# Kateridge/TransMF_AD

Measured on AMD Instinct MI355X. Metric: volume-pairs/sec fwd+bwd(+Adam), 96^3 MRI+PET batch=8 per GPU, higher is better.
Workload: dtype f32

## Files before the change

transmf_ad_amd/csrc/conv1_gram.hip:

```cpp
#include "tmf_common.h"

namespace {

constexpr int GT_D = 8, GT_H = 8, GT_W = 32;
constexpr int GP_D = GT_D + 2, GP_H = GT_H + 4, GP_W = GT_W + 4;
constexpr int GTHR = 512, GWG = 256, NACC = 64;

__host__ __device__ constexpr int kidx(int dd, int dh, int dw) {
    return dd == 0 ? (dh == 0 ? dw : 3 + (dh - 1) * 5 + (dw + 2)) : 13 + ((dd - 1) * 5 + (dh + 2)) * 5 + (dw + 2);
}
static_assert(kidx(2, 2, 2) == 62, "63 offsets");

typedef double f64x2 __attribute__((ext_vector_type(2)));
__device__ __forceinline__ float rbf16(float v) { return __builtin_bit_cast(float, tmf_pack_bf16(v, 0.f) << 16); }

__global__ __launch_bounds__(GTHR) void c1_gram_kernel(const float* __restrict__ x, double* __restrict__ part,
                                                        int D, int H, int W, int tilesD, int tilesH, int tilesW, int ntiles, int round16) {
    constexpr int NT = GP_D * GP_H * GP_W, NS = NT > 8 * GTHR ? NT : 8 * GTHR;
    __shared__ __attribute__((aligned(16))) double smem[NS];
    double* tile = smem;
    double* red = smem;
    const int tid = threadIdx.x;
    const int g = tid & 7, hh = (tid >> 3) & 7, dd0 = tid >> 6;
    double acc[63];
#pragma unroll
    for (int k = 0; k < 63; ++k) acc[k] = 0.0;
    double ssum = 0.0;
    constexpr int NE = (NT + GTHR - 1) / GTHR;
    int pe[NE];
#pragma unroll
    for (int j = 0; j < NE; ++j) {
        const int e = tid + j * GTHR;
        pe[j] = e < NT ? (e % GP_W) | (((e / GP_W) % GP_H) << 8) | ((e / (GP_W * GP_H)) << 16) : -1;
    }
    float pre[NE];
    auto fetch = [&](int t) {
        int r = t;
        const int bw = r % tilesW; r /= tilesW;
        const int bh = r % tilesH; r /= tilesH;
        const int bd = r % tilesD;
        const int b = r / tilesD;
        const int d0 = bd * GT_D, h0 = bh * GT_H - 2, w0 = bw * GT_W - 2;
        const float* xb = x + (size_t)b * D * H * W;
#pragma unroll
        for (int j = 0; j < NE; ++j) {
            const int gd = d0 + (pe[j] >> 16), gh = h0 + ((pe[j] >> 8) & 255), gw = w0 + (pe[j] & 255);
            float v = 0.f;
            if (pe[j] >= 0 && gd < D && gh >= 0 && gh < H && gw >= 0 && gw < W) v = xb[((size_t)gd * H + gh) * W + gw];
            pre[j] = round16 ? rbf16(v) : v;
        }
    };
    if ((int)blockIdx.x < ntiles) fetch(blockIdx.x);
    for (int t = blockIdx.x; t < ntiles; t += gridDim.x) {
        __syncthreads();
#pragma unroll
        for (int j = 0; j < NE; ++j)
            if (pe[j] >= 0) tile[tid + j * GTHR] = (double)pre[j];
        __syncthreads();
        if (t + (int)gridDim.x < ntiles) fetch(t + gridDim.x);
        const double* base = tile + (dd0 * GP_H + hh + 2) * GP_W + 4 * g;
        double a[4];
        {
            double rd[8];
#pragma unroll
            for (int j = 0; j < 4; ++j) { const f64x2 p = *reinterpret_cast<const f64x2*>(base + 2 * j); rd[2 * j] = p[0]; rd[2 * j + 1] = p[1]; }
            a[0] = rd[2]; a[1] = rd[3]; a[2] = rd[4]; a[3] = rd[5];
            ssum += (a[0] + a[1]) + (a[2] + a[3]);
#pragma unroll
            for (int dw = 0; dw <= 2; ++dw)
#pragma unroll
                for (int i = 0; i < 4; ++i) acc[kidx(0, 0, dw)] = fma(a[i], rd[i + 2 + dw], acc[kidx(0, 0, dw)]);
        }
#pragma unroll
        for (int dd = 0; dd <= 2; ++dd)
#pragma unroll
            for (int dh = -2; dh <= 2; ++dh) {
                if (dd == 0 && dh <= 0) continue;
                const double* row = base + (dd * GP_H + dh) * GP_W;
                double rd[8];
#pragma unroll
                for (int j = 0; j < 4; ++j) { const f64x2 p = *reinterpret_cast<const f64x2*>(row + 2 * j); rd[2 * j] = p[0]; rd[2 * j + 1] = p[1]; }
#pragma unroll
                for (int dw = -2; dw <= 2; ++dw)
#pragma unroll
                    for (int i = 0; i < 4; ++i) acc[kidx(dd, dh, dw)] = fma(a[i], rd[i + 2 + dw], acc[kidx(dd, dh, dw)]);
            }
    }
    const int lane = tid & 63, kq = tid >> 6;
#pragma unroll
    for (int c = 0; c < 8; ++c) {
        __syncthreads();
#pragma unroll
        for (int q = 0; q < 8; ++q) {
            const int k = c * 8 + q;
            red[q * GTHR + tid] = k < 63 ? acc[k < 63 ? k : 0] : ssum;
        }
        __syncthreads();
        double s = 0.0;
#pragma unroll
        for (int m = 0; m < 8; ++m) s += red[kq * GTHR + m * 64 + lane];
#pragma unroll
        for (int o = 32; o > 0; o >>= 1) s += __shfl_xor(s, o);
        if (lane == 0) part[(size_t)blockIdx.x * NACC + c * 8 + kq] = s;
    }
}

constexpr int GMAXC = 64;

constexpr int NGRAM = 760;
constexpr int HWG = 64, HTHR = 256, HNB = 288, HPART = 96;
constexpr int HNE = (HNB * 9 + HTHR - 1) / HTHR;

__host__ __device__ constexpr int class_tap(int cls, int j) {
    const int ax = cls >> 1, fixed = (cls & 1) ? 0 : 2, a = j / 3, b = j % 3;
    return ax == 0 ? fixed * 9 + a * 3 + b : (ax == 1 ? a * 9 + fixed * 3 + b : a * 9 + b * 3 + fixed);
}

__global__ __launch_bounds__(HTHR) void c1_shell_gram_kernel(const float* __restrict__ x, double* __restrict__ part, int B, int D, int H, int W,
                                                              int round16) {
    __shared__ double xs[HNB * 9];
    __shared__ int vbase[HNB], vcrd[HNB];
    __shared__ double red[3 * 81];
    const int tid = threadIdx.x, cls = blockIdx.y, ax = cls >> 1, side = cls & 1;
    const int n1 = ax == 0 ? H + 2 : D, n2 = ax == 2 ? H : W + 2;
    const int per = n1 * n2, total = B * per;
    const int p = tid % 81, slice = tid / 81, pi = p / 9, pj = p % 9;
    int cv_[HNE], cdd[HNE], cdh[HNE], cdw[HNE];
#pragma unroll
    for (int k = 0; k < HNE; ++k) {
        const int e = tid + k * HTHR, vi = e / 9, j = e - vi * 9, tap = class_tap(cls, j);
        cv_[k] = e < HNB * 9 ? vi : -1;
        cdd[k] = tap / 9 - 2; cdh[k] = (tap / 3) % 3 - 2; cdw[k] = tap % 3 - 2;
    }
    double acc = 0.0, eacc = 0.0;
    for (int base = blockIdx.x * HNB; base < total; base += gridDim.x * HNB) {
        __syncthreads();
        for (int vt = tid; vt < HNB; vt += HTHR) {
            const int s_ = base + vt;
            int c = -1, off = 0;
            if (s_ < total) {
                const int b = s_ / per, q = s_ - b * per, q1 = q / n2, q2 = q - q1 * n2;
                int vd, vh, vw;
                if (ax == 0) { vd = side ? D : -1; vh = q1 - 1; vw = q2 - 1; }
                else if (ax == 1) { vh = side ? H : -1; vd = q1; vw = q2 - 1; }
                else { vw = side ? W : -1; vd = q1; vh = q2; }
                c = (vd + 1) | (vh + 1) << 10 | (vw + 1) << 20;
                off = b * D * H * W;
            }
            vcrd[vt] = c; vbase[vt] = off;
        }
        __syncthreads();
#pragma unroll
        for (int k = 0; k < HNE; ++k) {
            if (cv_[k] < 0) continue;
            const int c = vcrd[cv_[k]];
            float v = 0.f;
            if (c >= 0) {
                const int ud = (c & 1023) + cdd[k], uh = ((c >> 10) & 1023) + cdh[k], uw = (c >> 20) + cdw[k];
                if (ud >= 0 && ud < D && uh >= 0 && uh < H && uw >= 0 && uw < W) v = x[(size_t)vbase[cv_[k]] + ((size_t)ud * H + uh) * W + uw];
            }
            xs[tid + k * HTHR] = (double)(round16 ? rbf16(v) : v);
        }
        __syncthreads();
        if (slice < 3) {
#pragma unroll 8
            for (int vi = slice * (HNB / 3); vi < (slice + 1) * (HNB / 3); ++vi) {
                const double xa = xs[vi * 9 + pi];
                acc = fma(xa, xs[vi * 9 + pj], acc);
                eacc += pj == 0 ? xa : 0.0;
            }
        }
    }
    __shared__ double rede[3 * 9];
    __syncthreads();
    if (slice < 3) {
        red[slice * 81 + p] = acc;
        if (pj == 0) rede[slice * 9 + pi] = eacc;
    }
    __syncthreads();
    double* row = part + ((size_t)cls * gridDim.x + blockIdx.x) * HPART;
    if (tid < 81) row[tid] = (red[tid] + red[81 + tid]) + red[162 + tid];
    else if (tid < 90) row[tid] = (rede[tid - 81] + rede[9 + tid - 81]) + rede[18 + tid - 81];
}

__global__ __launch_bounds__(1024) void c1_gram2_finish_kernel(const float* __restrict__ w, const double* __restrict__ rpart, int ngram,
                                                                const double* __restrict__ hpart, int nh, double* __restrict__ gram,
                                                                float* __restrict__ out, int C, int round16) {
    __shared__ double ra[16 * NACC];
    __shared__ double R[NACC];
    __shared__ double Hc[6 * HPART];
    __shared__ double G[27 * 27 + 27];
    __shared__ float wsh[27 * GMAXC];
    __shared__ double rows[27 * GMAXC];
    const int tid = threadIdx.x;
    {
        const int k = tid & 63, rg = tid >> 6;
        double s = 0.0;
#pragma unroll 8
        for (int i = rg; i < ngram; i += 16) s += rpart[(size_t)i * NACC + k];
        ra[rg * NACC + k] = s;
    }
    for (int e = tid; e < 27 * C; e += 1024) wsh[e] = round16 ? rbf16(w[e]) : w[e];
    for (int e = tid; e < 6 * HPART; e += 1024) {
        const int cls = e / HPART, k = e - cls * HPART;
        double s0 = 0.0, s1_ = 0.0, s2_ = 0.0, s3 = 0.0;
        if (k < 90) {
            int i = 0;
            for (; i + 3 < nh; i += 4) {
                s0 += hpart[((size_t)cls * nh + i) * HPART + k]; s1_ += hpart[((size_t)cls * nh + i + 1) * HPART + k];
                s2_ += hpart[((size_t)cls * nh + i + 2) * HPART + k]; s3 += hpart[((size_t)cls * nh + i + 3) * HPART + k];
            }
            for (; i < nh; ++i) s0 += hpart[((size_t)cls * nh + i) * HPART + k];
        }
        Hc[e] = (s0 + s1_) + (s2_ + s3);
    }
    __syncthreads();
    if (tid < NACC) {
        double s = 0.0;
#pragma unroll
        for (int i = 0; i < 16; ++i) s += ra[i * NACC + tid];
        R[tid] = s;
    }
    __syncthreads();
    for (int e = tid; e < 27 * 27 + 27; e += 1024) {
        double v;
        if (e < 729) {
            const int t = e / 27, u = e - t * 27;
            int dd = u / 9 - t / 9, dh = (u / 3) % 3 - (t / 3) % 3, dw = u % 3 - t % 3;
            if (dd < 0 || (dd == 0 && (dh < 0 || (dh == 0 && dw < 0)))) { dd = -dd; dh = -dh; dw = -dw; }
            v = R[kidx(dd, dh, dw)];
            for (int cls = 0; cls < 6; ++cls)
                for (int i = 0; i < 9; ++i) {
                    if (class_tap(cls, i) != t) continue;
                    for (int j = 0; j < 9; ++j)
                        if (class_tap(cls, j) == u) v -= Hc[cls * HPART + i * 9 + j];
// ... 49 lines not shown
    for (int e = tid; e < 27 * C; e += 1024) wsh[e] = round16 ? rbf16(w[e]) : w[e];
    __syncthreads();
    for (int j = tid; j < 2 * C; j += 1024) {
        double s = 0.0;
#pragma unroll
        for (int rg = 0; rg < 16; ++rg) s += pa[rg * 2 * C + j];
        c01[j] = s / count;
        if (coef) coef[j] = (float)c01[j];
        if (j < C) { if (dbeta) dbeta[j] = (float)s; }
        else if (dgamma) dgamma[j - C] = (float)s;
    }
    __syncthreads();
    for (int e = tid; e < 27 * C; e += 1024) {
        const int t = e / C, c = e - t * C;
        double v = 0.0;
        for (int u = 0; u < 27; ++u) v = fma((double)wsh[u * C + c], gram[t * 27 + u], v);
        const double st = gram[729 + t], mu = mean[c], is = invstd[c];
        const double r = (double)scale[c] * ((double)dred[e] - c01[c] * st - c01[C + c] * is * (v - mu * st));
        if (dw_ref) dw[(size_t)c * 27 + t] = (float)r;
        else dw[e] = (float)r;
    }
}

int c1_gram_mode() { return tmf_opt(TMF_OPT_C1_GRAM); }

}

extern "C" size_t tmf_c1_gram_bytes(int B, int D, int H, int W, int C) {
    if (B <= 0 || D <= 0 || H <= 0 || W <= 0 || C <= 0 || !c1_gram_mode() || C > GMAXC) return 0;
    if ((long)B * D * H * W >= (1L << 31) || D >= 1022 || H >= 1022 || W >= 1022) return 0;
    if ((long)B * tmf_cdiv(D, GT_D) * tmf_cdiv(H, GT_H) * tmf_cdiv(W, GT_W) >= (1L << 31)) return 0;
    return ((size_t)NGRAM + (size_t)GWG * NACC + (size_t)6 * HWG * HPART) * 8;
}
extern "C" size_t tmf_c1_gram_bytes_bf16(int B, int D, int H, int W, int C) {
    return c1_gram_mode() == 2 ? tmf_c1_gram_bytes(B, D, H, W, C) : 0;
}

static int c1_stats_g(int round16, const float* x, const float* w, float* stat_partial, void* gram, size_t gram_bytes,
                      int B, int D, int H, int W, int C, void* stream) {
    TMF_REQUIRE_PTR(x); TMF_REQUIRE_PTR(w); TMF_REQUIRE_PTR(stat_partial); TMF_REQUIRE_PTR(gram);
    const size_t need = tmf_c1_gram_bytes(B, D, H, W, C);
    TMF_REQUIRE(need > 0, TMF_E_SHAPE, "tmf_c1_stats_g: not available for this shape / option (tmf_c1_gram_bytes() = 0)");
    TMF_REQUIRE(gram_bytes >= need, TMF_E_WORKSPACE, "tmf_c1_stats_g: gram buffer %zu B < required %zu B", gram_bytes, need);
    TMF_REQUIRE((long)B * D * H * W < (1L << 31) && D < 1022 && H < 1022 && W < 1022, TMF_E_SHAPE,
                "tmf_c1_stats_g: the batch exceeds 2^31 voxels or an axis 1021");
    const int tilesD = tmf_cdiv(D, GT_D), tilesH = tmf_cdiv(H, GT_H), tilesW = tmf_cdiv(W, GT_W);
    const long ntiles = (long)B * tilesD * tilesH * tilesW;
    TMF_REQUIRE(ntiles < (1L << 31), TMF_E_SHAPE, "tmf_c1_stats_g: too many bricks");
    const int ngram = (int)(ntiles < GWG ? ntiles : GWG);
    double* g = (double*)gram;
    double* rpart = g + NGRAM;
    double* hpart = rpart + (size_t)GWG * NACC;
    hipStream_t s = (hipStream_t)stream;
    hipLaunchKernelGGL(c1_gram_kernel, dim3(ngram), dim3(GTHR), 0, s, x, rpart, D, H, W, tilesD, tilesH, tilesW, (int)ntiles, round16);
    hipLaunchKernelGGL(c1_shell_gram_kernel, dim3(HWG, 6), dim3(HTHR), 0, s, x, hpart, B, D, H, W, round16);
    hipLaunchKernelGGL(c1_gram2_finish_kernel, dim3(1), dim3(1024), 0, s, w, (const double*)rpart, ngram, (const double*)hpart, HWG, g,
                       stat_partial, C, round16);
    return tmf_launch_result("tmf_c1_stats_g");
}
extern "C" int tmf_c1_stats_g(const float* x, const float* w, float* stat_partial, void* gram, size_t gram_bytes,
                              int B, int D, int H, int W, int C, void* stream) {
    return c1_stats_g(0, x, w, stat_partial, gram, gram_bytes, B, D, H, W, C, stream);
}
extern "C" int tmf_c1_stats_g_bf16(const float* x, const float* w, float* stat_partial, void* gram, size_t gram_bytes,
                                   int B, int D, int H, int W, int C, void* stream) {
    return c1_stats_g(1, x, w, stat_partial, gram, gram_bytes, B, D, H, W, C, stream);
}

int tmf_c1_bwd_fused_finish(const float* part, int nblk, const float* dred, const float* w, const void* gram, const float* scale,
                            const float* mean, const float* invstd, double count, float* dgamma, float* dbeta, float* dw, int C,
                            int dw_ref, int round16, void* stream, float* coef) {
    hipLaunchKernelGGL(c1_bwd_fused_finish_kernel, dim3(1), dim3(1024), 0, (hipStream_t)stream, part, nblk, dred, w, (const double*)gram,
                       scale, mean, invstd, count, dgamma, dbeta, dw, C, dw_ref, round16, coef);
    return tmf_launch_result("tmf_c1_bwd_fused(finish)");
}
```

transmf_ad_amd/csrc/token_gemm.hip:

```cpp
#include <type_traits>
#include "tmf_device.h"

namespace {

constexpr int TM = 16, TTHR = 256;

struct TokArgs {
    const float* A; const float* W; float* Y;
    int R, K, N;
    const float* ln_g; const float* ln_b; float eps; float* ln_mean; float* ln_rstd; float* ln_out;
    const float* bias; const float* res; float* pre;
    const float* gelu_h;
    const float* lnb_x; const float* lnb_mean; const float* lnb_rstd; const float* lnb_g;
    const float* add1; const float* add2;
    float* lnb_partial; float* colsum_partial; int partial_stride;
    const float* mask; float* Y2;
};

__device__ __forceinline__ float hsum(f32x4 v) { return v[0] + v[1] + v[2] + v[3]; }
__device__ __forceinline__ float hsum(f32x2 v) { return v[0] + v[1]; }
__device__ __forceinline__ f32x4 minus(f32x4 v, float mu) { return f32x4{v[0] - mu, v[1] - mu, v[2] - mu, v[3] - mu}; }
__device__ __forceinline__ f32x2 minus(f32x2 v, float mu) { return f32x2{v[0] - mu, v[1] - mu}; }
__device__ __forceinline__ float sumsq(f32x4 d) { return d[0] * d[0] + d[1] * d[1] + d[2] * d[2] + d[3] * d[3]; }
__device__ __forceinline__ float sumsq(f32x2 d) { return d[0] * d[0] + d[1] * d[1]; }
// ... 323 lines not shown
        if (masked) TMF_REQUIRE_PTR_FN(fn, dx_masked);
        a.lnb_x = ln_x; a.lnb_mean = ln_mean; a.lnb_rstd = ln_rstd; a.lnb_g = ln_gamma;
        if (K == 64) return launch_ln_bwd<1>(a, s, fn);
        if (K == 128) return launch_ln_bwd<2>(a, s, fn);
        return launch_ln_bwd<4>(a, s, fn);
    }
    if (gelu) {
        TMF_REQUIRE(!masked || (add1 == nullptr && add2 == nullptr && dx_masked == nullptr), TMF_E_SHAPE,
                    "%s: the GELU-gradient epilogue takes no add1, add2 or dx_masked", fn);
        return launch_wide_opt_mask<true, 0, EPI_GELU_GRAD>(a, s, fn, "(gelu)");
    }
    a.res = add1;
    TMF_REQUIRE(add2 == nullptr, TMF_E_SHAPE, "%s: add2 needs the LayerNorm epilogue", fn);
    return launch_wide<true, 0, EPI_PLAIN>(a, s, fn, "");
}

extern "C" int tmf_tok_linear_fwd(const float* x, const float* w, const float* bias, const float* residual, float* y,
                                  int R, int K, int Nout, const float* ln_gamma, const float* ln_beta, float eps,
                                  float* ln_mean, float* ln_rstd, float* ln_out, float* gelu_pre, void* stream) {
    return tmf_tok_linear_fwd_impl(x, w, bias, residual, y, R, K, Nout, ln_gamma, ln_beta, eps, ln_mean, ln_rstd, ln_out, gelu_pre,
                                   nullptr, stream);
}

extern "C" int tmf_tok_linear_bwd_input(const float* dy, const float* w, float* dx, int R, int Nout, int K,
                                        const float* gelu_pre, const float* ln_x, const float* ln_mean,
                                        const float* ln_rstd, const float* ln_gamma, const float* add1,
                                        const float* add2, float* ln_partial, float* bias_partial,
                                        int partial_stride, void* stream) {
    return tmf_tok_linear_bwd_input_impl(dy, w, dx, R, Nout, K, gelu_pre, ln_x, ln_mean, ln_rstd, ln_gamma, add1, add2, ln_partial,
                                         bias_partial, partial_stride, nullptr, nullptr, stream);
}

extern "C" int tmf_tok_linear_fwd_masked(const float* x, const float* w, const float* bias, const float* residual, float* y,
                                         int R, int K, int Nout, const float* ln_gamma, const float* ln_beta, float eps,
                                         float* ln_mean, float* ln_rstd, float* ln_out, float* gelu_pre, const float* mask,
                                         void* stream) {
    TMF_REQUIRE_PTR(x); TMF_REQUIRE_PTR(w); TMF_REQUIRE_PTR(y); TMF_REQUIRE_PTR(mask);
    return tmf_tok_linear_fwd_impl(x, w, bias, residual, y, R, K, Nout, ln_gamma, ln_beta, eps, ln_mean, ln_rstd, ln_out, gelu_pre,
                                   mask, stream);
}

extern "C" int tmf_tok_linear_bwd_input_masked(const float* dy, const float* w, float* dx, int R, int Nout, int K,
                                               const float* gelu_pre, const float* ln_x, const float* ln_mean,
                                               const float* ln_rstd, const float* ln_gamma, const float* add1,
                                               const float* add2, float* ln_partial, float* bias_partial,
                                               int partial_stride, const float* mask, float* dx_masked, void* stream) {
    TMF_REQUIRE_PTR(dy); TMF_REQUIRE_PTR(w); TMF_REQUIRE_PTR(dx); TMF_REQUIRE_PTR(mask);
    return tmf_tok_linear_bwd_input_impl(dy, w, dx, R, Nout, K, gelu_pre, ln_x, ln_mean, ln_rstd, ln_gamma, add1, add2, ln_partial,
                                         bias_partial, partial_stride, mask, dx_masked, stream);
}

namespace {

constexpr int WG_MAXP = 32, WG_NSPLIT = 8;
struct WgMulti {
    const float* dy[WG_MAXP]; const float* x[WG_MAXP]; float* dw[WG_MAXP];
    int R[WG_MAXP], N[WG_MAXP], K[WG_MAXP], tile0[WG_MAXP + 1], elem0[WG_MAXP + 1];
    int nprob;
};

__global__ __launch_bounds__(256, 2) void tok_wgrad_multi_kernel(const WgMulti p, float* __restrict__ partial, long total_elems) {
    __shared__ float red[3][32 * 32];
    const int tid = threadIdx.x, lane = tid & 63;
    const int wave = __builtin_amdgcn_readfirstlane(tid >> 6);
    const int l31 = lane & 31, hsel = lane >> 5;
    int q = 0;
    while (q + 1 < p.nprob && (int)blockIdx.x >= p.tile0[q + 1]) ++q;
    const int t = blockIdx.x - p.tile0[q];
    const int tiles_k = p.K[q] >> 5;
    const int n0 = (t / tiles_k) * 32, k0 = (t % tiles_k) * 32;
    const int R = p.R[q], N = p.N[q], K = p.K[q];
    int rows = (R + WG_NSPLIT - 1) / WG_NSPLIT;
    rows = (rows + 7) & ~7;
    const int rb = blockIdx.y * rows + wave * (rows >> 2);
    const float* dy = p.dy[q] + n0 + l31;
    const float* xx = p.x[q] + k0 + l31;
    f32x16 acc;
#pragma unroll
    for (int r = 0; r < 16; ++r) acc[r] = 0.f;
    const int steps = rows >> 3;
    constexpr int UB = 16;
    for (int s0 = 0; s0 < steps; s0 += UB) {
        float a[UB], b[UB];
#pragma unroll
        for (int u = 0; u < UB; ++u) {
            const int row = rb + 2 * (s0 + u) + hsel;
            const bool ok = (s0 + u) < steps && row < R;
            const int rr = ok ? row : 0;
            a[u] = dy[(size_t)rr * N];
            b[u] = xx[(size_t)rr * K];
            a[u] = ok ? a[u] : 0.f;
        }
#pragma unroll
        for (int u = 0; u < UB; ++u) acc = __builtin_amdgcn_mfma_f32_32x32x2f32(a[u], b[u], acc, 0, 0, 0);
    }
    if (wave > 0) {
#pragma unroll
        for (int r = 0; r < 16; ++r) red[wave - 1][((r & 3) + 8 * (r >> 2) + 4 * hsel) * 32 + l31] = acc[r];
    }
    __syncthreads();
    if (wave == 0) {
        float* dst = partial + (size_t)blockIdx.y * total_elems + p.elem0[q];
#pragma unroll
        for (int r = 0; r < 16; ++r) {
            const int i = (r & 3) + 8 * (r >> 2) + 4 * hsel;
            const float v = acc[r] + red[0][i * 32 + l31] + red[1][i * 32 + l31] + red[2][i * 32 + l31];
            dst[(size_t)(n0 + i) * K + k0 + l31] = v;
        }
    }
}

__global__ __launch_bounds__(256) void tok_wgrad_multi_reduce_kernel(const WgMulti p, const float* __restrict__ partial,
                                                                     long total_elems) {
    const long e = (long)blockIdx.x * 256 + threadIdx.x;
    if (e >= total_elems) return;
    float s = 0.f;
#pragma unroll
    for (int k = 0; k < WG_NSPLIT; ++k) s += partial[(size_t)k * total_elems + e];
    int q = 0;
    while (q + 1 < p.nprob && e >= p.elem0[q + 1]) ++q;
    p.dw[q][e - p.elem0[q]] = s;
}

int fill_multi(WgMulti& m, int nprob, const float* const* dy, const float* const* x, float* const* dw,
               const int* R, const int* N, const int* K, const char* fn) {
    TMF_REQUIRE(nprob > 0 && nprob <= WG_MAXP, TMF_E_SHAPE, "%s: 1..%d problems, got %d", fn, WG_MAXP, nprob);
    m.nprob = nprob;
    m.tile0[0] = 0; m.elem0[0] = 0;
    for (int q = 0; q < nprob; ++q) {
        TMF_REQUIRE(R[q] > 0 && N[q] > 0 && K[q] > 0 && N[q] % 32 == 0 && K[q] % 32 == 0, TMF_E_SHAPE,
                    "%s: problem %d: R=%d N=%d K=%d (N and K must be multiples of 32)", fn, q, R[q], N[q], K[q]);
        m.R[q] = R[q]; m.N[q] = N[q]; m.K[q] = K[q];
        if (dy) { m.dy[q] = dy[q]; m.x[q] = x[q]; m.dw[q] = dw[q]; }
        m.tile0[q + 1] = m.tile0[q] + (N[q] / 32) * (K[q] / 32);
        m.elem0[q + 1] = m.elem0[q] + N[q] * K[q];
    }
    return TMF_OK;
}

}

extern "C" size_t tmf_tok_wgrad_multi_workspace_bytes(int nprob, const int* N, const int* K) {
    if (nprob <= 0 || nprob > WG_MAXP || N == nullptr || K == nullptr) return 0;
    size_t e = 0;
    for (int q = 0; q < nprob; ++q) e += (size_t)N[q] * K[q];
    return e * WG_NSPLIT * 4;
}

extern "C" int tmf_tok_wgrad_multi(int nprob, const float* const* dy, const float* const* x, float* const* dw,
                                   const int* R, const int* N, const int* K, void* workspace, size_t workspace_bytes,
                                   void* stream) {
    TMF_REQUIRE_PTR(dy); TMF_REQUIRE_PTR(x); TMF_REQUIRE_PTR(dw); TMF_REQUIRE_PTR(R); TMF_REQUIRE_PTR(N); TMF_REQUIRE_PTR(K);
    TMF_REQUIRE_PTR(workspace);
    WgMulti m = {};
    int rc = fill_multi(m, nprob, dy, x, dw, R, N, K, "tmf_tok_wgrad_multi");
    if (rc) return rc;
    for (int q = 0; q < nprob; ++q) { TMF_REQUIRE_PTR(dy[q]); TMF_REQUIRE_PTR(x[q]); TMF_REQUIRE_PTR(dw[q]); }
    const size_t need = tmf_tok_wgrad_multi_workspace_bytes(nprob, N, K);
    TMF_REQUIRE(workspace_bytes >= need, TMF_E_WORKSPACE, "tmf_tok_wgrad_multi: workspace %zu B < required %zu B",
                workspace_bytes, need);
    const long total = m.elem0[nprob];
    hipStream_t s = (hipStream_t)stream;
    hipLaunchKernelGGL(tok_wgrad_multi_kernel, dim3(m.tile0[nprob], WG_NSPLIT), dim3(256), 0, s, m, (float*)workspace, total);
    if ((rc = tmf_launch_result("tmf_tok_wgrad_multi"))) return rc;
    hipLaunchKernelGGL(tok_wgrad_multi_reduce_kernel, dim3((unsigned)tmf_cdiv(total, 256L)), dim3(256), 0, s, m,
                       (const float*)workspace, total);
    return tmf_launch_result("tmf_tok_wgrad_multi(reduce)");
}
```

transmf_ad_amd/csrc/token_ops.hip:

```cpp
#include "tmf_device.h"

static thread_local char g_err[512] = "";

void tmf_set_error(const char* fmt, ...) {
    va_list ap;
    va_start(ap, fmt);
    vsnprintf(g_err, sizeof g_err, fmt, ap);
    va_end(ap);
}

extern "C" int tmf_version(void) { return 1; }
extern "C" const char* tmf_last_error_string(void) { return g_err; }

namespace {

constexpr int LN_MAXV = 8;

template <int VEC>
__global__ __launch_bounds__(256) void layernorm_fwd_kernel(
    const float* __restrict__ x, const float* __restrict__ gamma, const float* __restrict__ beta,
    const float* __restrict__ residual, float* __restrict__ y, float* __restrict__ mean, float* __restrict__ rstd,
    int rows, int dim, float eps) {
    const int lane = threadIdx.x & 63;
    const int row = blockIdx.x * 4 + (threadIdx.x >> 6);
// ... 53 lines not shown
                    s1 += g;
                    s2 += g * xh;
                    ag[u * VEC + q] += gr[i + q] * xh;
                    ab[u * VEC + q] += gr[i + q];
                }
            }
        }
        s1 = wave_sum(s1) / dim;
        s2 = wave_sum(s2) / dim;
        float* dr = dx + (size_t)row * dim;
#pragma unroll
        for (int u = 0; u < LN_MAXV; ++u) {
            const int i = (u * 64 + lane) * VEC;
            if (i < dim) {
#pragma unroll
                for (int q = 0; q < VEC; ++q) {
                    const float xh = (xr[i + q] - mu) * rs;
                    const float v = rs * (gr[i + q] * gamma[i + q] - s1 - xh * s2);
                    dr[i + q] = v;
                    if (MASK) dxm[(size_t)row * dim + i + q] = v * mask[(size_t)row * dim + i + q];
                }
            }
        }
    }
#pragma unroll
    for (int u = 0; u < LN_MAXV; ++u) {
        const int i = (u * 64 + lane) * VEC;
        if (i < dim) {
#pragma unroll
            for (int q = 0; q < VEC; ++q) {
                red[(wave * 2 + 0) * dim + i + q] = ag[u * VEC + q];
                red[(wave * 2 + 1) * dim + i + q] = ab[u * VEC + q];
            }
        }
    }
    __syncthreads();
    for (int e = threadIdx.x; e < 2 * dim; e += 256) {
        const float a = red[e] + red[2 * dim + e] + red[4 * dim + e] + red[6 * dim + e];
        partial[(size_t)blockIdx.x * 2 * dim + e] = a;
    }
}

__global__ __launch_bounds__(256) void mask_mul_kernel(const float* __restrict__ x, const float* __restrict__ mask,
                                                       float* __restrict__ y, long n) {
    const long i = ((long)blockIdx.x * 256 + threadIdx.x) * 4;
    if (i + 4 <= n) {
        const f32x4 a = *reinterpret_cast<const f32x4*>(x + i), m = *reinterpret_cast<const f32x4*>(mask + i);
        *reinterpret_cast<f32x4*>(y + i) = f32x4{a[0] * m[0], a[1] * m[1], a[2] * m[2], a[3] * m[3]};
    } else {
        for (long j = i; j < n; ++j) y[j] = x[j] * mask[j];
    }
}

__global__ __launch_bounds__(256) void token_pool_fwd_kernel(const float* __restrict__ mri, const float* __restrict__ pet,
                                                             float* __restrict__ cls, int32_t* __restrict__ argmax,
                                                             int B, int N, int dim) {
    __shared__ float ssum[4][64], smax[4][64];
    __shared__ int sarg[4][64];
    const int cgroups = (dim + 63) / 64;
    const int cg = blockIdx.x % cgroups, mod = (blockIdx.x / cgroups) % 2, b = blockIdx.x / (2 * cgroups);
    const int cl = threadIdx.x & 63, tl = threadIdx.x >> 6;
    const int c = cg * 64 + cl;
    float s = 0.f, mx = -INFINITY;
    int am = 0;
    if (c < dim) {
        const float* src = (mod == 0 ? mri : pet) + (size_t)b * N * dim + c;
        for (int n = tl; n < N; n += 4) {
            const float v = src[(size_t)n * dim];
            s += v;
            if (v > mx || v != v) { mx = v; am = n; }
        }
    }
    ssum[tl][cl] = s; smax[tl][cl] = mx; sarg[tl][cl] = am;
    __syncthreads();
    if (tl == 0 && c < dim) {
#pragma unroll
        for (int k = 1; k < 4; ++k) {
            s += ssum[k][cl];
            const float v = smax[k][cl];
            const int a = sarg[k][cl];
            if (v != v) {
                if (mx == mx || a > am) { mx = v; am = a; }
            } else if (mx == mx && (v > mx || (v == mx && a < am))) { mx = v; am = a; }
        }
        cls[(size_t)b * 4 * dim + mod * dim + c] = s / N;
        cls[(size_t)b * 4 * dim + (2 + mod) * dim + c] = mx;
        argmax[((size_t)b * 2 + mod) * dim + c] = am;
    }
}

__global__ void token_pool_bwd_kernel(const float* __restrict__ dcls, const int32_t* __restrict__ argmax,
                                      float* __restrict__ dmri, float* __restrict__ dpet, int B, int N, int dim) {
    const long i = (long)blockIdx.x * blockDim.x + threadIdx.x;
    const long total = (long)B * 2 * N * dim;
    if (i >= total) return;
    const int c = i % dim;
    const int n = (i / dim) % N;
    const int mod = (i / ((long)dim * N)) % 2;
    const int b = i / ((long)dim * N * 2);
    const float gavg = dcls[(size_t)b * 4 * dim + mod * dim + c];
    const float gmax = dcls[(size_t)b * 4 * dim + (2 + mod) * dim + c];
    const int am = argmax[((size_t)b * 2 + mod) * dim + c];
    float* dst = (mod == 0 ? dmri : dpet);
    dst[((size_t)b * N + n) * dim + c] = gavg / N + (n == am ? gmax : 0.f);
}

__global__ __launch_bounds__(256) void pack_conv_weights_kernel(const float* __restrict__ w, float* __restrict__ fwd,
                                                                float* __restrict__ dgrad, int cout, int cin, int T) {
    const long n = (long)cout * cin * T;
    long e = (long)blockIdx.x * 256 + threadIdx.x;
    if (fwd != nullptr) {
        if (e < n) {
            const int co = e % cout, ci = (e / cout) % cin, t = e / ((long)cout * cin);
            fwd[e] = w[((long)co * cin + ci) * T + t];
            return;
        }
        e -= n;
    }
    if (dgrad != nullptr && e < n) {
        const int ci = e % cin, co = (e / cin) % cout, tr = e / ((long)cout * cin);
        dgrad[e] = w[((long)co * cin + ci) * T + (T - 1 - tr)];
    }
}

__global__ __launch_bounds__(256) void pack_conv_weights_bf16_kernel(const float* __restrict__ w, unsigned int* __restrict__ fwd,
                                                                     unsigned int* __restrict__ dgrad, int cout, int cin, int T) {
    const long n2 = (long)cout * cin * T / 2;
    long p = (long)blockIdx.x * 256 + threadIdx.x;
    if (p < n2) {
        const long e = 2 * p;
// ... 122 lines not shown

extern "C" int tmf_layernorm_bwd_blocks(int rows, int dim) {
    (void)dim;
    if (rows <= 0) return 0;
    return tmf_cdiv(rows, ln_rows_per_block(rows));
}

int tmf_layernorm_bwd_impl(const float* x, const float* gamma, const float* mean, const float* rstd, const float* dy, float* dx,
                           float* partial, int rows, int dim, const float* mask, float* dx_masked, void* stream) {
    const char* fn = mask != nullptr ? "tmf_layernorm_bwd_masked" : "tmf_layernorm_bwd";
    TMF_REQUIRE_PTR_FN(fn, x); TMF_REQUIRE_PTR_FN(fn, gamma); TMF_REQUIRE_PTR_FN(fn, mean); TMF_REQUIRE_PTR_FN(fn, rstd);
    TMF_REQUIRE_PTR_FN(fn, dy); TMF_REQUIRE_PTR_FN(fn, dx); TMF_REQUIRE_PTR_FN(fn, partial);
    if (mask != nullptr) TMF_REQUIRE_PTR_FN(fn, dx_masked);
    TMF_REQUIRE(rows > 0 && dim > 0, TMF_E_SHAPE, "%s: rows=%d dim=%d", fn, rows, dim);
    const int vec = dim % 4 == 0 ? 4 : 1;
    TMF_REQUIRE(dim <= 64 * vec * LN_MAXV, TMF_E_SHAPE, "%s: dim=%d exceeds %d", fn, dim, 64 * vec * LN_MAXV);
    const int rpb = ln_rows_per_block(rows);
    dim3 grid(tmf_cdiv(rows, rpb)), block(256);
    const size_t lds = (size_t)8 * dim * 4;
    if (mask == nullptr) dx_masked = nullptr;
    auto launch = [&](auto kernel) {
        hipLaunchKernelGGL(kernel, grid, block, lds, (hipStream_t)stream, x, gamma, mean, rstd, dy, dx, partial, rows, dim, rpb, mask, dx_masked);
    };
    if (mask != nullptr) vec == 4 ? launch(layernorm_bwd_kernel<4, true>) : launch(layernorm_bwd_kernel<1, true>);
    else                 vec == 4 ? launch(layernorm_bwd_kernel<4, false>) : launch(layernorm_bwd_kernel<1, false>);
    return tmf_launch_result(fn);
}

extern "C" int tmf_layernorm_bwd(const float* x, const float* gamma, const float* mean, const float* rstd,
                                 const float* dy, float* dx, float* partial, int rows, int dim, void* stream) {
    return tmf_layernorm_bwd_impl(x, gamma, mean, rstd, dy, dx, partial, rows, dim, nullptr, nullptr, stream);
}

extern "C" int tmf_layernorm_bwd_masked(const float* x, const float* gamma, const float* mean, const float* rstd,
                                        const float* dy, float* dx, float* partial, int rows, int dim,
                                        const float* mask, float* dx_masked, void* stream) {
    TMF_REQUIRE_PTR(x); TMF_REQUIRE_PTR(gamma); TMF_REQUIRE_PTR(mean); TMF_REQUIRE_PTR(rstd);
    TMF_REQUIRE_PTR(dy); TMF_REQUIRE_PTR(dx); TMF_REQUIRE_PTR(partial); TMF_REQUIRE_PTR(mask);
    return tmf_layernorm_bwd_impl(x, gamma, mean, rstd, dy, dx, partial, rows, dim, mask, dx_masked, stream);
}

extern "C" int tmf_mask_mul(const float* x, const float* mask, float* y, long n, void* stream) {
    TMF_REQUIRE_PTR(x); TMF_REQUIRE_PTR(mask); TMF_REQUIRE_PTR(y);
    TMF_REQUIRE_ALIGNED(x); TMF_REQUIRE_ALIGNED(mask); TMF_REQUIRE_ALIGNED(y);
    TMF_REQUIRE(n > 0 && n < (1L << 40), TMF_E_SHAPE, "tmf_mask_mul: n=%ld", n);
    hipLaunchKernelGGL(mask_mul_kernel, dim3((unsigned)tmf_cdiv(n, 1024L)), dim3(256), 0, (hipStream_t)stream, x, mask, y, n);
    return tmf_launch_result("tmf_mask_mul");
}

extern "C" int tmf_token_pool_fwd(const float* mri, const float* pet, float* cls, int32_t* argmax,
                                  int B, int N, int dim, void* stream) {
    TMF_REQUIRE_PTR(mri); TMF_REQUIRE_PTR(pet); TMF_REQUIRE_PTR(cls); TMF_REQUIRE_PTR(argmax);
    TMF_REQUIRE(B > 0 && N > 0 && dim > 0, TMF_E_SHAPE, "tmf_token_pool_fwd: B=%d N=%d dim=%d", B, N, dim);
    hipLaunchKernelGGL(token_pool_fwd_kernel, dim3(B * 2 * tmf_cdiv(dim, 64)), dim3(256), 0, (hipStream_t)stream,
                       mri, pet, cls, argmax, B, N, dim);
    return tmf_launch_result("tmf_token_pool_fwd");
}

extern "C" int tmf_token_pool_bwd(const float* dcls, const int32_t* argmax, float* dmri, float* dpet,
                                  int B, int N, int dim, void* stream) {
    TMF_REQUIRE_PTR(dcls); TMF_REQUIRE_PTR(argmax); TMF_REQUIRE_PTR(dmri); TMF_REQUIRE_PTR(dpet);
    TMF_REQUIRE(B > 0 && N > 0 && dim > 0, TMF_E_SHAPE, "tmf_token_pool_bwd: B=%d N=%d dim=%d", B, N, dim);
    const long total = (long)B * 2 * N * dim;
    hipLaunchKernelGGL(token_pool_bwd_kernel, dim3(tmf_cdiv(total, 256)), dim3(256), 0, (hipStream_t)stream,
                       dcls, argmax, dmri, dpet, B, N, dim);
    return tmf_launch_result("tmf_token_pool_bwd");
}
```

Baseline: 1029.

## Fuse conv1 gram kernels, retile token wgrad with LDS double-buffering, widen token pooling

The conv1 interior-gram and shell-gram kernels are merged into one launch. Its workgroups take either role, with each 512-thread group running two shell workgroups, so the two stages overlap and one launch is saved. The token weight-gradient GEMM moves to 64x64 tiles staged through double-buffered LDS with vectorized loads. Its split-K count is now adaptive, and the reduce pass is skipped when there is no split. Token pooling uses more threads per channel group with batched loads to raise memory-level parallelism. The changes raise LDS use and code complexity in exchange.

```diff
diff --git a/transmf_ad_amd/csrc/conv1_gram.hip b/transmf_ad_amd/csrc/conv1_gram.hip
--- a/transmf_ad_amd/csrc/conv1_gram.hip
+++ b/transmf_ad_amd/csrc/conv1_gram.hip
@@ -14,10 +14,15 @@
 typedef double f64x2 __attribute__((ext_vector_type(2)));
 __device__ __forceinline__ float rbf16(float v) { return __builtin_bit_cast(float, tmf_pack_bf16(v, 0.f) << 16); }
 
-__global__ __launch_bounds__(GTHR) void c1_gram_kernel(const float* __restrict__ x, double* __restrict__ part,
-                                                        int D, int H, int W, int tilesD, int tilesH, int tilesW, int ntiles, int round16) {
-    constexpr int NT = GP_D * GP_H * GP_W, NS = NT > 8 * GTHR ? NT : 8 * GTHR;
-    __shared__ __attribute__((aligned(16))) double smem[NS];
+constexpr int G_NT = GP_D * GP_H * GP_W, G_NS = G_NT > 8 * GTHR ? G_NT : 8 * GTHR;
+constexpr int HNB = 288;
+constexpr int H_NS = HNB * 9 + HNB + 3 * 81 + 3 * 9;
+constexpr int GS_NS = G_NS > 2 * H_NS ? G_NS : 2 * H_NS;
+
+__device__ __forceinline__ void c1_gram_role(double* __restrict__ smem, int blk, int nblk, const float* __restrict__ x,
+                                             double* __restrict__ part, int D, int H, int W, int tilesD, int tilesH, int tilesW,
+                                             int ntiles, int round16) {
+    constexpr int NT = G_NT;
     double* tile = smem;
     double* red = smem;
     const int tid = threadIdx.x;
@@ -50,14 +55,14 @@
             pre[j] = round16 ? rbf16(v) : v;
         }
     };
-    if ((int)blockIdx.x < ntiles) fetch(blockIdx.x);
-    for (int t = blockIdx.x; t < ntiles; t += gridDim.x) {
+    if (blk < ntiles) fetch(blk);
+    for (int t = blk; t < ntiles; t += nblk) {
         __syncthreads();
 #pragma unroll
         for (int j = 0; j < NE; ++j)
             if (pe[j] >= 0) tile[tid + j * GTHR] = (double)pre[j];
         __syncthreads();
-        if (t + (int)gridDim.x < ntiles) fetch(t + gridDim.x);
+        if (t + nblk < ntiles) fetch(t + nblk);
         const double* base = tile + (dd0 * GP_H + hh + 2) * GP_W + 4 * g;
         double a[4];
         {
@@ -101,27 +106,32 @@
         for (int m = 0; m < 8; ++m) s += red[kq * GTHR + m * 64 + lane];
 #pragma unroll
         for (int o = 32; o > 0; o >>= 1) s += __shfl_xor(s, o);
-        if (lane == 0) part[(size_t)blockIdx.x * NACC + c * 8 + kq] = s;
+        if (lane == 0) part[(size_t)blk * NACC + c * 8 + kq] = s;
     }
 }
 
 constexpr int GMAXC = 64;
 
 constexpr int NGRAM = 760;
-constexpr int HWG = 64, HTHR = 256, HNB = 288, HPART = 96;
+constexpr int HWG = 64, HTHR = 256, HPART = 96;
 constexpr int HNE = (HNB * 9 + HTHR - 1) / HTHR;
+static_assert(GTHR == 2 * HTHR && HWG % 2 == 0, "a 512-thread workgroup of the launch is a pair of shell workgroups");
 
 __host__ __device__ constexpr int class_tap(int cls, int j) {
     const int ax = cls >> 1, fixed = (cls & 1) ? 0 : 2, a = j / 3, b = j % 3;
     return ax == 0 ? fixed * 9 + a * 3 + b : (ax == 1 ? a * 9 + fixed * 3 + b : a * 9 + b * 3 + fixed);
 }
 
-__global__ __launch_bounds__(HTHR) void c1_shell_gram_kernel(const float* __restrict__ x, double* __restrict__ part, int B, int D, int H, int W,
-                                                              int round16) {
-    __shared__ double xs[HNB * 9];
-    __shared__ int vbase[HNB], vcrd[HNB];
-    __shared__ double red[3 * 81];
-    const int tid = threadIdx.x, cls = blockIdx.y, ax = cls >> 1, side = cls & 1;
+__device__ __forceinline__ void c1_shell_role(double* __restrict__ smem, int cls, int pair, const float* __restrict__ x,
+                                              double* __restrict__ part, int B, int D, int H, int W, int round16) {
+    const int half = threadIdx.x / HTHR, blk = 2 * pair + half;
+    smem += half * H_NS;
+    double* xs = smem;
+    int* vbase = reinterpret_cast<int*>(smem + HNB * 9);
+    int* vcrd = vbase + HNB;
+    double* red = smem + HNB * 9 + HNB;
+    double* rede = red + 3 * 81;
+    const int tid = threadIdx.x % HTHR, ax = cls >> 1, side = cls & 1;
     const int n1 = ax == 0 ? H + 2 : D, n2 = ax == 2 ? H : W + 2;
     const int per = n1 * n2, total = B * per;
     const int p = tid % 81, slice = tid / 81, pi = p / 9, pj = p % 9;
@@ -133,9 +143,11 @@
         cdd[k] = tap / 9 - 2; cdh[k] = (tap / 3) % 3 - 2; cdw[k] = tap % 3 - 2;
     }
     double acc = 0.0, eacc = 0.0;
-    for (int base = blockIdx.x * HNB; base < total; base += gridDim.x * HNB) {
-        __syncthreads();
-        for (int vt = tid; vt < HNB; vt += HTHR) {
+    for (int base0 = 2 * pair * HNB; base0 < total; base0 += HWG * HNB) {
+        const int base = base0 + half * HNB;
+        const bool live = base < total;
+        __syncthreads();
+        for (int vt = tid; live && vt < HNB; vt += HTHR) {
             const int s_ = base + vt;
             int c = -1, off = 0;
             if (s_ < total) {
@@ -150,19 +162,24 @@
             vcrd[vt] = c; vbase[vt] = off;
         }
         __syncthreads();
-#pragma unroll
-        for (int k = 0; k < HNE; ++k) {
-            if (cv_[k] < 0) continue;
-            const int c = vcrd[cv_[k]];
-            float v = 0.f;
-            if (c >= 0) {
+        if (live) {
+            float gv[HNE];
+            bool gok[HNE];
+#pragma unroll
+            for (int k = 0; k < HNE; ++k) {
+                const int vi = cv_[k] < 0 ? 0 : cv_[k], c = vcrd[vi];
                 const int ud = (c & 1023) + cdd[k], uh = ((c >> 10) & 1023) + cdh[k], uw = (c >> 20) + cdw[k];
-                if (ud >= 0 && ud < D && uh >= 0 && uh < H && uw >= 0 && uw < W) v = x[(size_t)vbase[cv_[k]] + ((size_t)ud * H + uh) * W + uw];
-            }
-            xs[tid + k * HTHR] = (double)(round16 ? rbf16(v) : v);
-        }
-        __syncthreads();
-        if (slice < 3) {
+                gok[k] = cv_[k] >= 0 && c >= 0 && ud >= 0 && ud < D && uh >= 0 && uh < H && uw >= 0 && uw < W;
+                gv[k] = x[gok[k] ? (size_t)vbase[vi] + ((size_t)ud * H + uh) * W + uw : (size_t)0];
+            }
+#pragma unroll
+            for (int k = 0; k < HNE; ++k) {
+                const float v = gok[k] ? gv[k] : 0.f;
+                if (cv_[k] >= 0) xs[tid + k * HTHR] = (double)(round16 ? rbf16(v) : v);
+            }
+        }
+        __syncthreads();
+        if (live && slice < 3) {
 #pragma unroll 8
             for (int vi = slice * (HNB / 3); vi < (slice + 1) * (HNB / 3); ++vi) {
                 const double xa = xs[vi * 9 + pi];
@@ -171,16 +188,24 @@
             }
         }
     }
-    __shared__ double rede[3 * 9];
     __syncthreads();
     if (slice < 3) {
         red[slice * 81 + p] = acc;
         if (pj == 0) rede[slice * 9 + pi] = eacc;
     }
     __syncthreads();
-    double* row = part + ((size_t)cls * gridDim.x + blockIdx.x) * HPART;
+    double* row = part + ((size_t)cls * HWG + blk) * HPART;
     if (tid < 81) row[tid] = (red[tid] + red[81 + tid]) + red[162 + tid];
     else if (tid < 90) row[tid] = (rede[tid - 81] + rede[9 + tid - 81]) + rede[18 + tid - 81];
+}
+
+__global__ __launch_bounds__(GTHR) void c1_gram_kernel_and_c1_shell_gram_kernel(const float* __restrict__ x, double* __restrict__ rpart,
+                                                              double* __restrict__ hpart, int B, int D, int H, int W, int tilesD,
+                                                              int tilesH, int tilesW, int ntiles, int ngram, int round16) {
+    __shared__ __attribute__((aligned(16))) double smem[GS_NS];
+    const int bid = blockIdx.x;
+    if (bid < 3 * HWG) c1_shell_role(smem, bid / (HWG / 2), bid % (HWG / 2), x, hpart, B, D, H, W, round16);
+    else c1_gram_role(smem, bid - 3 * HWG, ngram, x, rpart, D, H, W, tilesD, tilesH, tilesW, ntiles, round16);
 }
 
 __global__ __launch_bounds__(1024) void c1_gram2_finish_kernel(const float* __restrict__ w, const double* __restrict__ rpart, int ngram,
@@ -336,8 +361,8 @@
     double* rpart = g + NGRAM;
     double* hpart = rpart + (size_t)GWG * NACC;
     hipStream_t s = (hipStream_t)stream;
-    hipLaunchKernelGGL(c1_gram_kernel, dim3(ngram), dim3(GTHR), 0, s, x, rpart, D, H, W, tilesD, tilesH, tilesW, (int)ntiles, round16);
-    hipLaunchKernelGGL(c1_shell_gram_kernel, dim3(HWG, 6), dim3(HTHR), 0, s, x, hpart, B, D, H, W, round16);
+    hipLaunchKernelGGL(c1_gram_kernel_and_c1_shell_gram_kernel, dim3(3 * HWG + ngram), dim3(GTHR), 0, s, x, rpart, hpart, B, D, H, W, tilesD, tilesH, tilesW,
+                       (int)ntiles, ngram, round16);
     hipLaunchKernelGGL(c1_gram2_finish_kernel, dim3(1), dim3(1024), 0, s, w, (const double*)rpart, ngram, (const double*)hpart, HWG, g,
                        stat_partial, C, round16);
     return tmf_launch_result("tmf_c1_stats_g");
diff --git a/transmf_ad_amd/csrc/token_gemm.hip b/transmf_ad_amd/csrc/token_gemm.hip
--- a/transmf_ad_amd/csrc/token_gemm.hip
+++ b/transmf_ad_amd/csrc/token_gemm.hip
@@ -399,74 +399,133 @@
 
 namespace {
 
-constexpr int WG_MAXP = 32, WG_NSPLIT = 8;
+constexpr int WG_MAXP = 32, WG_MAXSPLIT = 8, WG_T = 64, WG_ROWS = 32;
+constexpr int WG_FILL = 4 * 256;
 struct WgMulti {
     const float* dy[WG_MAXP]; const float* x[WG_MAXP]; float* dw[WG_MAXP];
     int R[WG_MAXP], N[WG_MAXP], K[WG_MAXP], tile0[WG_MAXP + 1], elem0[WG_MAXP + 1];
     int nprob;
 };
 
-__global__ __launch_bounds__(256, 2) void tok_wgrad_multi_kernel(const WgMulti p, float* __restrict__ partial, long total_elems) {
-    __shared__ float red[3][32 * 32];
+int wg_splits(int tiles, int max_rows) {
+    int s = tmf_cdiv(WG_FILL, tiles);
+    if (s > WG_MAXSPLIT) s = WG_MAXSPLIT;
+    const int by_rows = tmf_cdiv(max_rows, WG_ROWS);
+    if (s > by_rows) s = by_rows;
+    return s < 1 ? 1 : s;
+}
+
+template <bool VEC>
+__global__ __launch_bounds__(256, 2) void tok_wgrad_multi_kernel(const WgMulti p, float* __restrict__ partial, long total_elems,
+                                                                 int nsplit) {
+    __shared__ __attribute__((aligned(16))) float sa[2][WG_ROWS][WG_T], sb[2][WG_ROWS][WG_T];
     const int tid = threadIdx.x, lane = tid & 63;
     const int wave = __builtin_amdgcn_readfirstlane(tid >> 6);
     const int l31 = lane & 31, hsel = lane >> 5;
+    const int item = blockIdx.x;
     int q = 0;
-    while (q + 1 < p.nprob && (int)blockIdx.x >= p.tile0[q + 1]) ++q;
-    const int t = blockIdx.x - p.tile0[q];
-    const int tiles_k = p.K[q] >> 5;
-    const int n0 = (t / tiles_k) * 32, k0 = (t % tiles_k) * 32;
+    while (q + 1 < p.nprob && item >= p.tile0[q + 1] * nsplit) ++q;
     const int R = p.R[q], N = p.N[q], K = p.K[q];
-    int rows = (R + WG_NSPLIT - 1) / WG_NSPLIT;
+    const int tiles_k = (K + WG_T - 1) / WG_T, tiles_q = p.tile0[q + 1] - p.tile0[q];
+    const int split = (item - p.tile0[q] * nsplit) / tiles_q, t = (item - p.tile0[q] * nsplit) % tiles_q;
+    const int n0 = (t / tiles_k) * WG_T, k0 = (t % tiles_k) * WG_T;
+    int rows = (R + nsplit - 1) / nsplit;
     rows = (rows + 7) & ~7;
-    const int rb = blockIdx.y * rows + wave * (rows >> 2);
-    const float* dy = p.dy[q] + n0 + l31;
-    const float* xx = p.x[q] + k0 + l31;
+    const int rb = split * rows;
+    const int re = rb + rows < R ? rb + rows : R;
+    const int wn = wave >> 1, wk = wave & 1;
+    const bool active = n0 + wn * 32 < N && k0 + wk * 32 < K;
+    const int lr = tid >> 4, lc = (tid & 15) * 4;
+    const float* dy = p.dy[q] + (n0 + lc < N ? n0 + lc : 0);
+    const float* xx = p.x[q] + (k0 + lc < K ? k0 + lc : 0);
+    auto fetch = [&](int r0, f32x4 (&va)[2], f32x4 (&vb)[2]) {
+#pragma unroll
+        for (int i = 0; i < 2; ++i) {
+            const int row = r0 + lr + 16 * i;
+            const size_t rr = row < R ? row : R - 1;
+            const float* pa = dy + rr * N;
+            const float* pb = xx + rr * K;
+            if constexpr (VEC) {
+                va[i] = *reinterpret_cast<const f32x4*>(pa);
+                vb[i] = *reinterpret_cast<const f32x4*>(pb);
+            } else {
+                va[i] = f32x4{pa[0], pa[1], pa[2], pa[3]};
+                vb[i] = f32x4{pb[0], pb[1], pb[2], pb[3]};
+            }
+        }
+    };
+    auto stash = [&](int buf, const f32x4 (&va)[2], const f32x4 (&vb)[2]) {
+#pragma unroll
+        for (int i = 0; i < 2; ++i) {
+            *reinterpret_cast<f32x4*>(&sa[buf][lr + 16 * i][lc]) = va[i];
+            *reinterpret_cast<f32x4*>(&sb[buf][lr + 16 * i][lc]) = vb[i];
+        }
+    };
     f32x16 acc;
 #pragma unroll
     for (int r = 0; r < 16; ++r) acc[r] = 0.f;
-    const int steps = rows >> 3;
-    constexpr int UB = 16;
-    for (int s0 = 0; s0 < steps; s0 += UB) {
-        float a[UB], b[UB];
-#pragma unroll
-        for (int u = 0; u < UB; ++u) {
-            const int row = rb + 2 * (s0 + u) + hsel;
-            const bool ok = (s0 + u) < steps && row < R;
-            const int rr = ok ? row : 0;
-            a[u] = dy[(size_t)rr * N];
-            b[u] = xx[(size_t)rr * K];
-            a[u] = ok ? a[u] : 0.f;
-        }
-#pragma unroll
-        for (int u = 0; u < UB; ++u) acc = __builtin_amdgcn_mfma_f32_32x32x2f32(a[u], b[u], acc, 0, 0, 0);
-    }
-    if (wave > 0) {
-#pragma unroll
-        for (int r = 0; r < 16; ++r) red[wave - 1][((r & 3) + 8 * (r >> 2) + 4 * hsel) * 32 + l31] = acc[r];
-    }
-    __syncthreads();
-    if (wave == 0) {
-        float* dst = partial + (size_t)blockIdx.y * total_elems + p.elem0[q];
-#pragma unroll
-        for (int r = 0; r < 16; ++r) {
-            const int i = (r & 3) + 8 * (r >> 2) + 4 * hsel;
-            const float v = acc[r] + red[0][i * 32 + l31] + red[1][i * 32 + l31] + red[2][i * 32 + l31];
-            dst[(size_t)(n0 + i) * K + k0 + l31] = v;
-        }
-    }
-}
-
+    auto multiply = [&](int buf, int r0) {
+        const int left = re - r0;
+        if (!active || left <= 0) return;
+        const int steps = left >= WG_ROWS ? WG_ROWS / 2 : (left + 1) >> 1;
+        const float* a = &sa[buf][hsel][wn * 32 + l31];
+        const float* b = &sb[buf][hsel][wk * 32 + l31];
+        if (steps == WG_ROWS / 2) {
+#pragma unroll
+            for (int s = 0; s < WG_ROWS / 2; ++s)
+                acc = __builtin_amdgcn_mfma_f32_32x32x2f32(a[2 * s * WG_T], b[2 * s * WG_T], acc, 0, 0, 0);
+        } else {
+            for (int s = 0; s < steps; ++s) {
+                const bool ok = 2 * s + hsel < left;
+                acc = __builtin_amdgcn_mfma_f32_32x32x2f32(ok ? a[2 * s * WG_T] : 0.f, ok ? b[2 * s * WG_T] : 0.f, acc, 0, 0, 0);
+            }
+        }
+    };
+    f32x4 va0[2], vb0[2], va1[2], vb1[2];
+    fetch(rb, va0, vb0);
+    __builtin_amdgcn_sched_barrier(0);
+    fetch(rb + WG_ROWS, va1, vb1);
+    __builtin_amdgcn_sched_barrier(0);
+    for (int r0 = rb; r0 < re; r0 += 2 * WG_ROWS) {
+        stash(0, va0, vb0);
+        __syncthreads();
+        fetch(r0 + 2 * WG_ROWS, va0, vb0);
+        multiply(0, r0);
+        stash(1, va1, vb1);
+        __syncthreads();
+        fetch(r0 + 3 * WG_ROWS, va1, vb1);
+        multiply(1, r0 + WG_ROWS);
+    }
+    if (active) {
+        float* dst = nsplit == 1 ? p.dw[q] : partial + (size_t)split * total_elems + p.elem0[q];
+        dst += (size_t)(n0 + wn * 32) * K + k0 + wk * 32 + l31;
+#pragma unroll
+        for (int r = 0; r < 16; ++r) dst[(size_t)((r & 3) + 8 * (r >> 2) + 4 * hsel) * K] = acc[r];
+    }
+}
+
+template <bool VEC>
 __global__ __launch_bounds__(256) void tok_wgrad_multi_reduce_kernel(const WgMulti p, const float* __restrict__ partial,
-                                                                     long total_elems) {
-    const long e = (long)blockIdx.x * 256 + threadIdx.x;
+                                                                     long total_elems, int nsplit) {
+    const long e = ((long)blockIdx.x * 256 + threadIdx.x) * 4;
     if (e >= total_elems) return;
-    float s = 0.f;
-#pragma unroll
-    for (int k = 0; k < WG_NSPLIT; ++k) s += partial[(size_t)k * total_elems + e];
+    f32x4 v[WG_MAXSPLIT];
+#pragma unroll
+    for (int k = 0; k < WG_MAXSPLIT; ++k) {
+        const float* src = partial + (size_t)(k < nsplit ? k : 0) * total_elems + e;
+        if constexpr (VEC) v[k] = *reinterpret_cast<const f32x4*>(src);
+        else v[k] = f32x4{src[0], src[1], src[2], src[3]};
+    }
+    f32x4 s = v[0];
+#pragma unroll
+    for (int k = 1; k < WG_MAXSPLIT; ++k)
+        if (k < nsplit) s += v[k];
+    const long e0 = (long)blockIdx.x * 1024;
     int q = 0;
-    while (q + 1 < p.nprob && e >= p.elem0[q + 1]) ++q;
-    p.dw[q][e - p.elem0[q]] = s;
+    while (q + 1 < p.nprob && e0 >= p.elem0[q + 1]) ++q;
+    float* dst = p.dw[q] + (e - p.elem0[q]);
+    if constexpr (VEC) *reinterpret_cast<f32x4*>(dst) = s;
+    else { dst[0] = s[0]; dst[1] = s[1]; dst[2] = s[2]; dst[3] = s[3]; }
 }
 
 int fill_multi(WgMulti& m, int nprob, const float* const* dy, const float* const* x, float* const* dw,
@@ -479,7 +538,7 @@
                     "%s: problem %d: R=%d N=%d K=%d (N and K must be multiples of 32)", fn, q, R[q], N[q], K[q]);
         m.R[q] = R[q]; m.N[q] = N[q]; m.K[q] = K[q];
         if (dy) { m.dy[q] = dy[q]; m.x[q] = x[q]; m.dw[q] = dw[q]; }
-        m.tile0[q + 1] = m.tile0[q] + (N[q] / 32) * (K[q] / 32);
+        m.tile0[q + 1] = m.tile0[q] + tmf_cdiv(N[q], WG_T) * tmf_cdiv(K[q], WG_T);
         m.elem0[q + 1] = m.elem0[q] + N[q] * K[q];
     }
     return TMF_OK;
@@ -490,8 +549,14 @@
 extern "C" size_t tmf_tok_wgrad_multi_workspace_bytes(int nprob, const int* N, const int* K) {
     if (nprob <= 0 || nprob > WG_MAXP || N == nullptr || K == nullptr) return 0;
     size_t e = 0;
-    for (int q = 0; q < nprob; ++q) e += (size_t)N[q] * K[q];
-    return e * WG_NSPLIT * 4;
+    int tiles = 0;
+    for (int q = 0; q < nprob; ++q) {
+        if (N[q] <= 0 || K[q] <= 0) return 0;
+        e += (size_t)N[q] * K[q];
+        tiles += tmf_cdiv(N[q], WG_T) * tmf_cdiv(K[q], WG_T);
+    }
+    const int ns = wg_splits(tiles, 1 << 30);
+    return ns > 1 ? e * ns * 4 : 16;
 }
 
 extern "C" int tmf_tok_wgrad_multi(int nprob, const float* const* dy, const float* const* x, float* const* dw,
@@ -502,15 +567,23 @@
     WgMulti m = {};
     int rc = fill_multi(m, nprob, dy, x, dw, R, N, K, "tmf_tok_wgrad_multi");
     if (rc) return rc;
-    for (int q = 0; q < nprob; ++q) { TMF_REQUIRE_PTR(dy[q]); TMF_REQUIRE_PTR(x[q]); TMF_REQUIRE_PTR(dw[q]); }
+    int vec = 1, dw_vec = (reinterpret_cast<uintptr_t>(workspace) & 15u) == 0, max_rows = 0;
+    for (int q = 0; q < nprob; ++q) {
+        TMF_REQUIRE_PTR(dy[q]); TMF_REQUIRE_PTR(x[q]); TMF_REQUIRE_PTR(dw[q]);
+        if ((reinterpret_cast<uintptr_t>(dy[q]) | reinterpret_cast<uintptr_t>(x[q])) & 15u) vec = 0;
+        if (reinterpret_cast<uintptr_t>(dw[q]) & 15u) dw_vec = 0;
+        if (R[q] > max_rows) max_rows = R[q];
+    }
     const size_t need = tmf_tok_wgrad_multi_workspace_bytes(nprob, N, K);
     TMF_REQUIRE(workspace_bytes >= need, TMF_E_WORKSPACE, "tmf_tok_wgrad_multi: workspace %zu B < required %zu B",
                 workspace_bytes, need);
     const long total = m.elem0[nprob];
+    const int nsplit = wg_splits(m.tile0[nprob], max_rows);
     hipStream_t s = (hipStream_t)stream;
-    hipLaunchKernelGGL(tok_wgrad_multi_kernel, dim3(m.tile0[nprob], WG_NSPLIT), dim3(256), 0, s, m, (float*)workspace, total);
-    if ((rc = tmf_launch_result("tmf_tok_wgrad_multi"))) return rc;
-    hipLaunchKernelGGL(tok_wgrad_multi_reduce_kernel, dim3((unsigned)tmf_cdiv(total, 256L)), dim3(256), 0, s, m,
-                       (const float*)workspace, total);
+    hipLaunchKernelGGL(vec ? tok_wgrad_multi_kernel<true> : tok_wgrad_multi_kernel<false>, dim3(m.tile0[nprob] * nsplit), dim3(256), 0, s,
+                       m, (float*)workspace, total, nsplit);
+    if ((rc = tmf_launch_result("tmf_tok_wgrad_multi")) || nsplit == 1) return rc;
+    hipLaunchKernelGGL(dw_vec ? tok_wgrad_multi_reduce_kernel<true> : tok_wgrad_multi_reduce_kernel<false>,
+                       dim3((unsigned)tmf_cdiv(total, 1024L)), dim3(256), 0, s, m, (const float*)workspace, total, nsplit);
     return tmf_launch_result("tmf_tok_wgrad_multi(reduce)");
 }
diff --git a/transmf_ad_amd/csrc/token_ops.hip b/transmf_ad_amd/csrc/token_ops.hip
--- a/transmf_ad_amd/csrc/token_ops.hip
+++ b/transmf_ad_amd/csrc/token_ops.hip
@@ -129,30 +129,42 @@
     }
 }
 
-__global__ __launch_bounds__(256) void token_pool_fwd_kernel(const float* __restrict__ mri, const float* __restrict__ pet,
-                                                             float* __restrict__ cls, int32_t* __restrict__ argmax,
-                                                             int B, int N, int dim) {
-    __shared__ float ssum[4][64], smax[4][64];
-    __shared__ int sarg[4][64];
-    const int cgroups = (dim + 63) / 64;
+constexpr int TP_CH = 32, TP_TL = 16, TP_PB = 8;
+__global__ __launch_bounds__(TP_CH * TP_TL) void token_pool_fwd_kernel(const float* __restrict__ mri, const float* __restrict__ pet,
+                                                                       float* __restrict__ cls, int32_t* __restrict__ argmax,
+                                                                       int B, int N, int dim) {
+    __shared__ float ssum[TP_TL][TP_CH], smax[TP_TL][TP_CH];
+    __shared__ int sarg[TP_TL][TP_CH];
+    const int cgroups = (dim + TP_CH - 1) / TP_CH;
     const int cg = blockIdx.x % cgroups, mod = (blockIdx.x / cgroups) % 2, b = blockIdx.x / (2 * cgroups);
-    const int cl = threadIdx.x & 63, tl = threadIdx.x >> 6;
-    const int c = cg * 64 + cl;
+    const int cl = threadIdx.x % TP_CH, tl = threadIdx.x / TP_CH;
+    const int c = cg * TP_CH + cl;
     float s = 0.f, mx = -INFINITY;
     int am = 0;
     if (c < dim) {
         const float* src = (mod == 0 ? mri : pet) + (size_t)b * N * dim + c;
-        for (int n = tl; n < N; n += 4) {
-            const float v = src[(size_t)n * dim];
-            s += v;
-            if (v > mx || v != v) { mx = v; am = n; }
+        for (int n0 = tl; n0 < N; n0 += TP_TL * TP_PB) {
+            float v[TP_PB];
+#pragma unroll
+            for (int u = 0; u < TP_PB; ++u) {
+                const int n = n0 + u * TP_TL;
+                v[u] = src[(size_t)(n < N ? n : N - 1) * dim];
+            }
+#pragma unroll
+            for (int u = 0; u < TP_PB; ++u) {
+                const int n = n0 + u * TP_TL;
+                if (n < N) {
+                    s += v[u];
+                    if (v[u] > mx || v[u] != v[u]) { mx = v[u]; am = n; }
+                }
+            }
         }
     }
     ssum[tl][cl] = s; smax[tl][cl] = mx; sarg[tl][cl] = am;
     __syncthreads();
     if (tl == 0 && c < dim) {
 #pragma unroll
-        for (int k = 1; k < 4; ++k) {
+        for (int k = 1; k < TP_TL; ++k) {
             s += ssum[k][cl];
             const float v = smax[k][cl];
             const int a = sarg[k][cl];
@@ -381,7 +393,7 @@
                                   int B, int N, int dim, void* stream) {
     TMF_REQUIRE_PTR(mri); TMF_REQUIRE_PTR(pet); TMF_REQUIRE_PTR(cls); TMF_REQUIRE_PTR(argmax);
     TMF_REQUIRE(B > 0 && N > 0 && dim > 0, TMF_E_SHAPE, "tmf_token_pool_fwd: B=%d N=%d dim=%d", B, N, dim);
-    hipLaunchKernelGGL(token_pool_fwd_kernel, dim3(B * 2 * tmf_cdiv(dim, 64)), dim3(256), 0, (hipStream_t)stream,
+    hipLaunchKernelGGL(token_pool_fwd_kernel, dim3(B * 2 * tmf_cdiv(dim, TP_CH)), dim3(TP_CH * TP_TL), 0, (hipStream_t)stream,
                        mri, pet, cls, argmax, B, N, dim);
     return tmf_launch_result("tmf_token_pool_fwd");
 }
```

Measured after the change: 1013. -1.5%, worse.
